# chennachaos/PFEMFort

Measured on AMD Instinct MI355X. Metric: DOF/s (assembly+CG-to-tol), higher is better.
Workload: dtype f64

## Files before the change

include/pfem_amd_diag.h:

```cpp
#ifndef PFEM_AMD_DIAG_H
#define PFEM_AMD_DIAG_H

#include "pfem_amd.h"

#ifdef __cplusplus
extern "C" {
#endif

#define PFEM_ASSEMBLY_GATHER 0
#define PFEM_ASSEMBLY_SCATTER 1
int pfem_solver_set_assembly_mode(pfem_solver *s, int mode);
int pfem_solver_assembly_info(pfem_solver *s, int *gather_form, int *hub_nodes, int *block_threads, int64_t *lds_bytes);
#define PFEM_SPMV_AUTO 0
#define PFEM_SPMV_INT32 1
#define PFEM_SPMV_GAPS16 2
#define PFEM_SPMV_GROUPED 3
int pfem_solver_set_spmv_format(pfem_solver *s, int format);
int pfem_solver_get_spmv_format(pfem_solver *s, int *bits_per_column);
int pfem_solver_get_spmv_row_group(pfem_solver *s, int *rows_per_lane);
int pfem_solver_get_spmv_gap_table(pfem_solver *s, int *entries);
int pfem_solver_get_spmv_value_dictionary(pfem_solver *s, int *entries);
int pfem_solver_amg_value_dictionaries(pfem_solver *s, int max_levels, int *n_levels, int *entries);
int pfem_solver_get_spmv_gap_escapes(pfem_solver *s, int *in_use);
int pfem_solver_spmv_bytes(pfem_solver *s, int64_t *format_bytes);

int pfem_solver_amg_info(pfem_solver *s, int max_levels, int *n_levels, int64_t *rows, int64_t *nnz, double *lambda_max,
                         double *symbolic_ms, double *numeric_ms, int *cheb_degree, int *fine_degree, double *eig_ratio, double *coarse_scale);
int pfem_solver_amg_aggregates(pfem_solver *s, int level, int32_t *agg);
int pfem_solver_amg_transfer(pfem_solver *s, int level, int *rbm, int *fine_bs, int *coarse_bs, int *dim, int64_t *n_nodes, double *node_xyz);
int pfem_solver_amg_layout(pfem_solver *s, int max_levels, int *coupled, int *distributed_levels, int64_t *first_dof, int64_t *local_rows);
int pfem_solver_incidence_patterns(pfem_solver *s, int *count, int *longest);
int pfem_solver_amg_aggregation(pfem_solver *s, int max_levels, int *n_levels, int *kind);
int pfem_solver_amg_comm_counts(pfem_solver *s, int *exchanges_per_cycle, int *allreduces_per_cycle);
int pfem_solver_amg_cycle_profile(pfem_solver *s, int max_levels, int *n_levels, int *exchanges, double *exchange_ms,
                                  int64_t *exchange_doubles, int *allreduces, double *allreduce_ms, int64_t *allreduce_doubles,
                                  double *cycle_ms);
int pfem_solver_amg_pairing(pfem_solver *s, int *lattice_levels);
int pfem_solver_amg_cycle(pfem_solver *s, int *cycle, int *last_level_visited_twice);
int pfem_solver_amg_level0_epilogue(pfem_solver *s, int *taken);

int pfem_eval_elems(pfem_solver *s, const double *elemData, const double *timeData,
                    double *K_out, double *F_out);

int pfem_matrix_info(pfem_solver *s, int64_t *n_owned, int64_t *n_local, int64_t *nnz,
                     int64_t *stored_entries);

int pfem_spmv(pfem_solver *s, const double *x, double *y);
int pfem_bench_spmv(pfem_solver *s, int reps, double *ms_per_launch);

typedef struct pfem_timings {
    double pattern_ms;
    double assemble_ms;
    double solve_ms;
    double spmv_ms_total;
    int64_t spmv_launches;
    double upload_ms;
    double event_overhead_ms;
    double iface_ms_total;
    double scalar_ms_total;
    int64_t comm_samples;
    double exposed_ms_total;
    int64_t graph_iterations;
// ... 21 lines not shown
```

pfemfort_amd/_lib.py:

```python
from __future__ import annotations

import ctypes as C
import os

_HERE = os.path.dirname(os.path.abspath(__file__))
LIB_PATH = os.environ.get("PFEM_AMD_LIB") or os.path.join(_HERE, "libpfem_amd.so")

OK, ERR_ARG, ERR_STATE, ERR_NEG_JAC, ERR_HIP, ERR_NOGPU, ERR_NOMEM, ERR_DIVERGED, ERR_PATTERN, ERR_COMM = range(10)
POISSON_TRIA, POISSON_TET, ELAST_TET, POISSON_TRIA_INLINE, ELAST_TRIA = 1, 2, 3, 4, 5
SOLVER_EMPTY, PATTERN_OK, INIT_OK, ASSEMBLY_OK, FACTORISE_OK = 1, 2, 3, 4, 5
INSERT_VALUES, ADD_VALUES = 1, 2

NPELEM = {POISSON_TRIA: 3, POISSON_TET: 4, ELAST_TET: 4, POISSON_TRIA_INLINE: 3, ELAST_TRIA: 3}
NDOF = {POISSON_TRIA: 1, POISSON_TET: 1, ELAST_TET: 3, POISSON_TRIA_INLINE: 1, ELAST_TRIA: 2}
NDIM = {POISSON_TRIA: 2, POISSON_TET: 3, ELAST_TET: 3, POISSON_TRIA_INLINE: 2, ELAST_TRIA: 2}


class PfemError(RuntimeError):
    def __init__(self, code: int, where: str, detail: str = ""):
        self.code = code
        msg = f"{where}: error {code} ({_strerror(code)})"
        if detail:
            msg += f" -- {detail}"
        super().__init__(msg)
# ... 68 lines not shown
    "pfem_solver_get_spmv_format": [_P, _P],
    "pfem_solver_get_spmv_row_group": [_P, _P],
    "pfem_solver_get_spmv_gap_table": [_P, _P],
    "pfem_solver_get_spmv_value_dictionary": [_P, _P],
    "pfem_solver_amg_value_dictionaries": [_P, _I, _P, _P],
    "pfem_solver_get_spmv_gap_escapes": [_P, _P],
    "pfem_solver_spmv_bytes": [_P, _P],
    "pfem_solver_set_preconditioner": [_P, _I],
    "pfem_solver_get_preconditioner": [_P, _P],
    "pfem_solver_set_cg_single_reduction": [_P, _I],
    "pfem_solver_amg_info": [_P, _I, _P, _P, _P, _P, _P, _P, _P, _P, _P, _P],
    "pfem_solver_amg_aggregates": [_P, _I, _P],
    "pfem_solver_amg_transfer": [_P, _I, _P, _P, _P, _P, _P, _P],
    "pfem_solver_amg_layout": [_P, _I, _P, _P, _P, _P],
    "pfem_solver_amg_aggregation": [_P, _I, _P, _P],
    "pfem_solver_incidence_patterns": [_P, _P, _P],
    "pfem_solver_amg_comm_counts": [_P, _P, _P],
    "pfem_solver_amg_cycle_profile": [_P, _I, _P, _P, _P, _P, _P, _P, _P, _P],
    "pfem_solver_amg_pairing": [_P, _P],
    "pfem_solver_set_amg_options": [_P, _I, _I, _D, _D],
    "pfem_solver_set_amg_cycle": [_P, _I],
    "pfem_solver_amg_cycle": [_P, _P, _P],
    "pfem_solver_amg_level0_epilogue": [_P, _P],
    "pfem_eval_elems": [_P, _P, _P, _P, _P],
    "pfem_rhs_add_values": [_P, _L, _P, _P],
    "pfem_matrix_info": [_P, _P, _P, _P, _P],
    "pfem_get_local_to_global": [_P, _P],
    "pfem_get_csr": [_P, _P, _P, _P],
    "pfem_get_rhs": [_P, _P],
    "pfem_spmv": [_P, _P, _P],
    "pfem_bench_spmv": [_P, _I, _P],
    "pfem_get_timings": [_P, _P],
    "pfem_solver_profile_spmv": [_P, _I],
    "pfem_neighbour_plan": [_I, _I, _P, _P, _P, _P, _P, _P, _P, _P, _P],
    "pfem_solver_set_neighbours": [_P, _I, _P, _P, _P],
    "pfem_rccl_unique_id": [_P],
    "pfem_solver_set_comm_rccl": [_P, _I, _I, _P],
    "pfem_solver_set_comm_host": [_P, _I, _I, HOST_ALLREDUCE_FN, HOST_EXCHANGE_FN, _P],
    "pfem_solver_comm_bench": [_P, C.c_int64, _I, _P, _P],
    "pfem_solver_comm_bench_sizes": [_P, C.c_int64, C.c_int64, _I, _I, _P, _P],
    "pfem_solver_set_comm_peer": [_P, _I, _I, HOST_ALLREDUCE_FN, HOST_EXCHANGE_FN, _P],
    "pfem_solver_comm_shutdown": [_P],
    "pfem_solver_comm_info": [_P, _P, _P, _P, _P],
    "pfem_solver_comm_describe": [_P, _P, _I, _P, _P, _P, _P, _P],
    "pfem_solver_comm_selftest": [_P, _L, _P],
    "pfem_get_ghosts": [_P, _P, _P],
# ... 53 lines not shown
```

pfemfort_amd/csrc/pfem_amg.inc:

```

constexpr int kAmgMaxLevels = 14;
constexpr int kAmgMatchRounds = 8;
constexpr int kAmgPasses = 3;
constexpr int64_t kAmgReplicateRows = 150000;
constexpr int kAmgRetryBlock = -7701;

inline bool amg_in_effect(const pfem_solver *s)
{
    return s->pc == PFEM_PC_GAMG;
}

inline SellDev amg_sell(const pfem_solver *s, const AmgLevel &L, int64_t rows)
{
    SellDev A;
    if (L.fine) {
        A = s->sell();
    } else {
        A.slice_off = L.slice_off.p;
        A.rowlen = L.rowlen.p;
        A.cols = L.cols.p;
        A.vals = L.vals.p;
    }
    A.n_rows = rows;
    A.n_slices = (rows + 63) / 64;
// ... 527 lines not shown
    const size_t n = static_cast<size_t>(std::max<int64_t>(L.n_loc, 1));
    const size_t g = L.fine ? static_cast<size_t>(kVecGuard) : 0;
    const size_t nv = n;
    PFEM_TRY(L.dinv.alloc(n));
    PFEM_TRY(L.t.alloc(nv));
    PFEM_TRY(L.r.alloc(n));
    if (!L.fine) PFEM_TRY(L.b.alloc(n));
    PFEM_TRY(L.x_store.alloc(nv + 2 * g));
    PFEM_TRY(L.dd_store.alloc(nv + 2 * g));
    PFEM_HIP(hipMemsetAsync(L.x_store.p, 0, sizeof(double) * (nv + 2 * g), s->stream));
    PFEM_HIP(hipMemsetAsync(L.dd_store.p, 0, sizeof(double) * (nv + 2 * g), s->stream));
    L.x = L.x_store.p + g;
    L.dd = L.dd_store.p + g;
    PFEM_TRY(L.lam.alloc(1));
    PFEM_TRY(L.part_max.alloc(static_cast<size_t>(grid_for((L.n_loc + 63) / 64 * 64))));
    return PFEM_OK;
}

inline bool amg_galerkin_by_entry()
{
    static const bool v = std::getenv("PFEM_AMG_GALERKIN_MAPS") != nullptr;
    return v;
}
inline void amg_galerkin(pfem_solver *s, const AmgLevel &L, AmgLevel &C, const SellDev &A, bool extras = false, VdState *vstate = nullptr)
{
    C.bound_fresh = C.vd_direct = false;
    if (L.code_of.p && !amg_galerkin_by_entry()) {
        if (C.n_loc < 1) return;
        LatGalExtra X{nullptr, nullptr, nullptr, nullptr, nullptr};
        if (extras && C.dinv.p && C.t.p && C.n_loc == C.n) {
            X.dinv_out = C.dinv.p;
            X.ratio_out = C.t.p;
            C.bound_fresh = true;
            if (vstate && C.vd_have_dict && C.vd_hash_ok && C.vhash.p && C.vcodes.p && C.vcodes.n >= static_cast<size_t>(C.stored) && !C.vd_refused) {
                const VdState reset{C.vd_n, 0, 0, 0};
                (void)hipMemcpyAsync(vstate, &reset, sizeof reset, hipMemcpyHostToDevice, s->stream);
                X.vhash = C.vhash.p;
                X.codes = C.vcodes.p;
                X.vstate = vstate;
                C.vd_direct = true;
            }
        }
        hipLaunchKernelGGL(k_lat_galerkin, dim3(static_cast<unsigned>((C.n_loc + kLatGalThreads - 1) / kLatGalThreads)), dim3(kLatGalThreads), 0, s->stream, A, C.n_loc,
                           static_cast<const int32_t *>(L.mem_ptr.p), static_cast<const int32_t *>(L.mem_idx.p), static_cast<const uint8_t *>(L.code_of.p),
                           static_cast<const uint32_t *>(L.code_mask.p), static_cast<const int64_t *>(C.slice_off.p), C.vals.p, X);
        return;
    }
    hipLaunchKernelGGL(k_amg_galerkin, dim3(grid_for(L.nnz_c)), dim3(kBlock), 0, s->stream, L.nnz_c, static_cast<const int64_t *>(L.src_ptr.p),
                       static_cast<const int32_t *>(L.src_slot.p), static_cast<const int64_t *>(L.dst_slot.p),
                       static_cast<const double *>(A.vals), C.vals.p);
}

int amg_couple_level(pfem_solver *s, AmgWork &W, AmgLevel &L, AmgLevel &C, bool overlap, int cb, const std::vector<double> *nc_of)
{
    std::vector<int64_t> rank_off;
    if (cb > 0 && nc_of) {
        rank_off.assign(nc_of->size() + 1, 0);
        for (size_t q = 0; q < nc_of->size(); ++q) rank_off[q + 1] = rank_off[q] + static_cast<int64_t>((*nc_of)[q]);
    }
    auto node_base = [&](int64_t g) -> int64_t {
        const size_t q = static_cast<size_t>(std::upper_bound(rank_off.begin(), rank_off.end(), g) - rank_off.begin()) - 1;
        return rank_off[q] + (g - rank_off[q]) / cb * cb;
    };
    const PlanRef P = amg_plan(s, L);
// ... 1985 lines not shown
        PFEM_TRY(check_kernel("k_vd_hash_build (coarse level)"));
        PFEM_TRY(encode(L, l));
    }
    PFEM_TRY(read_states());
    for (int l : build) {
        AmgLevel &L = *M.lev[static_cast<size_t>(l)];
        const VdState &v = st[static_cast<size_t>(l)];
        if (v.fail || v.count < 1 || v.count > kVdMax || v.miss) {
            L.vd_ok = L.vd_have_dict = L.vd_hash_ok = false;
            L.vd_refused = true;
        } else {
            L.vd_n = v.count;
            L.vd_have_dict = true;
            L.vd_ok = true;
            L.vd_hash_ok = L.vhash.p != nullptr;
        }
        if (std::getenv("PFEM_VD_VERBOSE"))
            std::fprintf(stderr, "  value dictionary, level %d: %d distinct values among %lld slots%s\n", l, v.count, static_cast<long long>(L.stored),
                         L.vd_ok ? "" : " -- the level keeps its fp64 values");
    }
    return PFEM_OK;
}

int amg_numeric(pfem_solver *s, Amg &M, bool overlap)
{
    if (M.coupled) return amg_numeric_coupled(s, M, overlap);
    const bool fresh = M.galerkin_fresh;
    M.galerkin_fresh = false;
    for (size_t l = 0; l < M.lev.size(); ++l) {
        AmgLevel &L = *M.lev[l];
        const SellDev A = amg_sell(s, L);
        if (l + 1 < M.lev.size() && !fresh) {
            AmgLevel &C = *M.lev[l + 1];
            if (L.rbm) amg_rbm_galerkin(s, L, C, A);
            else amg_galerkin(s, L, C, A, !M.rbm && !M.coupled, M.vd_states.p ? M.vd_states.p + (l + 1) : nullptr);
        }
        const unsigned g = grid_for(A.n_slices * 64);
        if (!L.fine && L.bound_fresh && !fresh) {
            L.bound_fresh = false;
            if (L.n > 65536) {
                const unsigned gm = std::min<unsigned>(g, 512u);
                hipLaunchKernelGGL(k_amg_max_rows, dim3(gm), dim3(kBlock), 0, s->stream, static_cast<const double *>(L.t.p), L.n, L.part_max.p);
                hipLaunchKernelGGL(k_amg_max, dim3(1), dim3(1024), 0, s->stream, static_cast<const double *>(L.part_max.p), static_cast<int64_t>(gm), L.lam.p);
            } else {
                hipLaunchKernelGGL(k_amg_max, dim3(1), dim3(1024), 0, s->stream, static_cast<const double *>(L.t.p), L.n, L.lam.p);
            }
            continue;
        }
        if (L.fine && s->asm_bound_fresh && &M == s->amg.get()) {
            const unsigned gm = std::min<unsigned>(g, 2048u);
            hipLaunchKernelGGL(k_amg_max_rows, dim3(gm), dim3(kBlock), 0, s->stream, static_cast<const double *>(L.t.p), L.n, L.part_max.p);
            hipLaunchKernelGGL(k_amg_max, dim3(1), dim3(1024), 0, s->stream, static_cast<const double *>(L.part_max.p), static_cast<int64_t>(gm), L.lam.p);
            s->asm_bound_fresh = false;
        } else {
        hipLaunchKernelGGL(k_amg_diag_bound, dim3(g), dim3(kBlock), 0, s->stream, A, static_cast<int32_t>(L.n), L.dinv.p, L.part_max.p);
        hipLaunchKernelGGL(k_amg_max, dim3(1), dim3(1024), 0, s->stream, static_cast<const double *>(L.part_max.p), static_cast<int64_t>(g), L.lam.p);
        }
        if (M.rbm) {
// ... 549 lines not shown
```

pfemfort_amd/csrc/pfem_amg_kernels.hpp:

```cpp
#pragma once

namespace pfem {

__device__ __forceinline__ int64_t amg_edge_key(int32_t i, int32_t j, int32_t hi_, int32_t hj_, double w, double di, double dj)
{
    if (!(w < 0.0) || !(di > 0.0) || !(dj > 0.0)) return -1;
    const double s = -w / sqrt(di * dj);
    int b = static_cast<int>(floor(8.0 * log2(s))) + 2048;
    b = b < 1 ? 1 : (b > 4095 ? 4095 : b);
    const int64_t lo = hi_ < hj_ ? hi_ : hj_, hi = hi_ < hj_ ? hj_ : hi_;
    const int64_t close = 0x7fffffffLL - (hi - lo);
    const int64_t par = (lo & 1) == 0;
    const int64_t a = i < j ? i : j, c = i < j ? j : i;
    const int64_t h = ((a * 2654435761LL + c * 40503LL) >> 7) & 0x7ffffLL;
    return (static_cast<int64_t>(b) << 51) | (close << 20) | (par << 19) | h;
}

__global__ void __launch_bounds__(kBlock) k_amg_match_pick(int64_t n, const int64_t *__restrict__ gptr, const int32_t *__restrict__ gcol,
                                                            const double *__restrict__ gw, const double *__restrict__ gdiag,
                                                            const int32_t *__restrict__ hint ,
                                                            const int32_t *__restrict__ match, int32_t *__restrict__ cand)
{
    const int64_t i = static_cast<int64_t>(blockIdx.x) * kBlock + threadIdx.x;
    if (i >= n) return;
// ... 406 lines not shown
    if (MAPS && I == na - 1) src_ptr[e] = p0 + run;
    uint32_t mask = 0;
    for (int32_t m = mem_ptr[I]; m < mem_ptr[I + 1]; ++m) {
        const int64_t i = mem_idx[m];
        const int64_t base = A.slice_off[i >> 6] + (i & 63);
        const int len = A.rowlen[i];
        for (int k = 0; k < len; ++k) {
            const int64_t q = base + 64LL * k;
            const int c = lat_code(B, pos[A.cols[q]], bix, biy, biz);
            if (MAPS) src_slot[p0 + at[c][t]++] = static_cast<int32_t>(q);
            code_of[q] = static_cast<uint8_t>(c);
            mask |= 1u << c;
        }
    }
    code_mask[I] = mask;
}
constexpr int kLatGalThreads = 128;
struct LatGalExtra {
    double *dinv_out, *ratio_out;
    const VdHashEntry *vhash;
    uint16_t *codes;
    VdState *vstate;
};
__global__ void __launch_bounds__(kLatGalThreads) k_lat_galerkin(SellDev A, int64_t na, const int32_t *__restrict__ mem_ptr,
                                                                  const int32_t *__restrict__ mem_idx, const uint8_t *__restrict__ code_of,
                                                                  const uint32_t *__restrict__ code_mask, const int64_t *__restrict__ c_slice_off,
                                                                  double *__restrict__ coarse_vals, LatGalExtra X)
{
    __shared__ double acc[kLatCodes][kLatGalThreads];
    const int64_t I = static_cast<int64_t>(blockIdx.x) * kLatGalThreads + threadIdx.x;
    if (I >= na) return;
    const int t = threadIdx.x;
#pragma unroll
    for (int c = 0; c < kLatCodes; ++c) acc[c][t] = 0.0;
    const int32_t m0 = mem_ptr[I], m1 = mem_ptr[I + 1];
    for (int32_t mb = m0; mb < m1; mb += 8) {
        int32_t mi[8];
        int len[8];
        int64_t base[8];
#pragma unroll
        for (int j = 0; j < 8; ++j) mi[j] = mb + j < m1 ? __builtin_nontemporal_load(mem_idx + mb + j) : -1;
#pragma unroll
        for (int j = 0; j < 8; ++j) {
            len[j] = mi[j] >= 0 ? A.rowlen[mi[j]] : 0;
            base[j] = mi[j] >= 0 ? A.slice_off[mi[j] >> 6] + (mi[j] & 63) : 0;
        }
#pragma unroll
        for (int j = 0; j < 8; ++j) {
            for (int k0 = 0; k0 < len[j]; k0 += 16) {
                double v[16];
                uint8_t c[16];
#pragma unroll
                for (int e = 0; e < 16; ++e) {
                    const bool in = k0 + e < len[j];
                    const int64_t q = base[j] + 64LL * (k0 + e);
                    v[e] = in ? __builtin_nontemporal_load(A.vals + q) : 0.0;
                    c[e] = in ? __builtin_nontemporal_load(code_of + q) : static_cast<uint8_t>(0);
                }
#pragma unroll
                for (int e = 0; e < 16; ++e)
                    if (k0 + e < len[j]) acc[c[e]][t] += v[e];
            }
        }
    }
    const int64_t out0 = c_slice_off[I >> 6] + (I & 63);
    double *out = coarse_vals + out0;
    const uint32_t mask = code_mask[I];
    int r = 0;
    double sabs = 0.0;
    bool missed = false;
#pragma unroll
    for (int c = 0; c < kLatCodes; ++c)
        if (mask & (1u << c)) {
            const double v = acc[c][t];
            out[64LL * r] = v;
            sabs += fabs(v);
            if (X.vhash) {
                int code = vd_hash_find(X.vhash, static_cast<unsigned long long>(__double_as_longlong(v)));
                if (code < 0) { missed = true; code = 0; }
                X.codes[out0 + 64LL * r] = static_cast<uint16_t>(code);
            }
            ++r;
        }
    if (X.dinv_out) {
        const double d = (mask & (1u << 13)) ? acc[13][t] : 0.0;
        const bool pos = d > 0.0;
        X.dinv_out[I] = pos ? 1.0 / d : 1.0;
        X.ratio_out[I] = pos ? sabs / d : 1.0;
    }
    if (missed) X.vstate->miss = 1;
}
constexpr int kLatticeTable = 4096;
__global__ void __launch_bounds__(kBlock) k_amg_distinct(const double *__restrict__ c, int64_t n, unsigned long long *__restrict__ table,
                                                          int *__restrict__ overflow)
{
    const int64_t i = static_cast<int64_t>(blockIdx.x) * kBlock + threadIdx.x;
    const double v = (i < n ? c[i] : 0.0) + 0.0;
    const unsigned long long key = static_cast<unsigned long long>(__double_as_longlong(v));
    const unsigned long long left = __shfl_up(key, 1, 64);
    if (i >= n || ((threadIdx.x & 63) != 0 && left == key && i - 1 < n)) return;
    if (key == ~0ull) { *overflow = 1; return; }
    unsigned h = static_cast<unsigned>((key * 0x9E3779B97F4A7C15ull) >> 52) & (kLatticeTable - 1);
    for (int probe = 0; probe < kLatticeTable; ++probe) {
        if ((probe & 63) == 0 && __hip_atomic_load(overflow, __ATOMIC_RELAXED, __HIP_MEMORY_SCOPE_AGENT) != 0) return;
        const unsigned long long cur = table[h];
        if (cur == key) return;
        if (cur == ~0ull) {
            const unsigned long long old = atomicCAS(&table[h], ~0ull, key);
            if (old == ~0ull || old == key) return;
        }
        h = (h + 1) & (kLatticeTable - 1);
    }
    *overflow = 1;
// ... 1341 lines not shown
```

pfemfort_amd/csrc/pfem_amg_types.hpp:

```cpp
#pragma once

struct AmgPlan {
    std::vector<int> peers;
    std::vector<int64_t> peer_off{0};
    std::vector<int32_t> send_lidx;
    int64_t n_send = 0, n_sh = 0;
    DevBuf<int32_t> d_send_lidx, d_sh_lidx, d_sh_ptr, d_sh_src;
    DevBuf<int32_t> d_row_sh;
};

struct AmgLevel {
    int64_t n = 0, n_slices = 0, stored = 0, nnz = 0;
    int64_t n_loc = 0;
    int64_t gid_off = 0;
    std::vector<int64_t> ghost_gid;
    AmgPlan plan;
    DevBuf<int32_t> gid;
    bool fine = false;
    DevBuf<int64_t> slice_off, rowptr;
    DevBuf<int32_t> rowlen, cols;
    DevBuf<double> vals;
    int bs = 1;
    int64_t n_nodes = 0;
    DevBuf<int32_t> node_of, comp_of;
// ... 4 lines not shown
    bool lat_global = false;
    std::vector<int> lat_cuts[3];
    std::vector<char> lat_single[3];
    int lat_shift[3] = {0, 0, 0};
    int lat_occ[6] = {0, 0, 0, 0, 0, 0};
    int lat_box[6] = {0, 0, 0, 0, 0, 0};
    bool lat_full = false;
    int lat_tlo[3] = {0, 0, 0}, lat_thi[3] = {0, 0, 0};
    bool lat_nodes_global = false;
    std::vector<std::pair<int, int>> lat_str[3];
    bool lat_split = false;
    std::vector<double> lat_coord;
    DevBuf<double> xyz;
    int agg_kind = 0;
    int64_t nc = 0;
    DevBuf<int32_t> agg;
    DevBuf<int32_t> mem_ptr, mem_idx;
    int64_t nnz_c = 0;
    DevBuf<int64_t> src_ptr;
    DevBuf<int32_t> src_slot;
    DevBuf<int64_t> dst_slot;
    DevBuf<uint8_t> code_of;
    DevBuf<uint32_t> code_mask;
    int dim = 0;
    bool rbm = false;
    DevBuf<double> cen;
    DevBuf<double> roff;
    DevBuf<int32_t> node_agg;
    DevBuf<int64_t> gptr;
    DevBuf<int32_t> gcol, brow;
    int64_t nblk = 0;
    DevBuf<double> dinv, t, r, b, x_store, dd_store, lam, part_max;
    DevBuf<uint16_t> vcodes;
    DevBuf<double> vdict;
    DevBuf<unsigned long long> vtable;
    int vd_n = 0;
    bool vd_ok = false, vd_have_dict = false, vd_refused = false;
    DevBuf<VdHashEntry> vhash;
    bool vd_hash_ok = false;
    bool vd_direct = false;
    bool bound_fresh = false;
    double *x = nullptr, *dd = nullptr;
    DevBuf<double> x1;
    double lam_host = 0.0;
};

// ... 4 lines not shown
    bool symbolic_ok = false;
    bool galerkin_fresh = false;
    double symbolic_ms = 0.0, numeric_ms = 0.0;
    int cheb_degree = 2;
    int fine_degree = 1;
    bool eig_ratio_given = false;
    bool coarse_scale_given = false;
    double eig_ratio_opt = 0.0, coarse_scale_opt = 0.0;
    double eig_ratio_auto = 16.0, coarse_scale_auto = 1.5;
    double eig_ratio = 8.0, coarse_scale = 1.5;
    CgGraph graph;
    hipEvent_t ev_num0 = nullptr, ev_num1 = nullptr;
    ~Amg()
    {
        if (ev_num0) (void)hipEventDestroy(ev_num0);
        if (ev_num1) (void)hipEventDestroy(ev_num1);
    }
    int tail_from = -1;
    size_t tail_lds_allowed = 0;
    int cycle_gamma = 1, w_to = -1;
    bool cycle_given = false;
    bool fused = true;
    bool level0_ep = false;
    int coarsest_sweeps = 8;
    bool coupled = false;
    bool coupled_fused = true;
    bool coupled_refused = false;
    int64_t n_last_global = 0;
    DevBuf<double> dense_glob, bx_glob, lam_all;
    std::unique_ptr<Amg> rep;
    DevBuf<double> rep_buf;
    DevBuf<int32_t> rep_pack_slot;
    int64_t rep_total = 0, rep_off = 0, rep_mine = 0;
    bool rbm = false;
    DevBuf<double> lam2;
    DevBuf<VdState> vd_states;
    int cycle_exchanges = 0, cycle_allreduces = 0;
};
```

pfemfort_amd/csrc/pfem_device.hip:

```cpp
#include <hip/hip_runtime.h>
#include <hip/hip_ext.h>
#include <hipcub/hipcub.hpp>
#include <rccl/rccl.h>
#include <dlfcn.h>

#include <algorithm>
#include <chrono>
#include <climits>
#include <cmath>
#include <cstdio>
#include <cstdlib>
#include <cstring>
#include <mutex>
#include <thread>
#include <string>
#include <deque>
#include <functional>
#include <map>
#include <memory>
#include <vector>

#include "pfem_internal.hpp"
#include "pfem_vdhash.hpp"
#include "pfem_kernels.hpp"
// ... 478 lines not shown
    bool use_grouped() const
    {
        return grouped && (spmv_format == PFEM_SPMV_GROUPED || (spmv_format == PFEM_SPMV_AUTO && n_groups >= min_groups_auto()));
    }
    bool relgrouped = false;
    bool rel_gap32 = false;
    bool rel_dict = false;
    DevBuf<uint32_t> d_gap_table;
    bool row_dict = false;
    DevBuf<uint32_t> d_row_gap_table;
    int64_t n_rgroups = 0, n_rslices = 0, r_stored = 0;
    DevBuf<int32_t> d_rcol0;
    DevBuf<int64_t> d_rslice_off, d_rslice_doff;
    DevBuf<uint32_t> d_rdwords;
    DevBuf<double> d_rvals;
    DevBuf<uint8_t> d_relk;
    bool rel_vals_current = false;
    bool asm_bound_fresh = false;
    DevBuf<int32_t> d_row_group;
    bool grp_vals_current = false;
    DevBuf<unsigned long long> d_vcodes, d_vtable;
    DevBuf<VdHashEntry> d_vhash;
    bool vd_hash_ok = false, vd_direct_pending = false;
    VdState vd_direct_verdict{0, 0, 1, 0};
    DevBuf<double> d_vdict;
    DevBuf<VdState> d_vstate;
    int vd_rows = 0, vd_n = 0;
    bool vd_current = false, vd_ok = false, vd_have_dict = false;
    double vd_encode_ms = 0.0;
    DevBuf<uint16_t> d_dcodes;
    DevBuf<double> d_ddict;
    DevBuf<unsigned long long> d_dtable;
    DevBuf<VdState> d_dstate;
    bool dinv_codes = false;
    DinvView dinv_view() const
    {
        return dinv_codes ? DinvView{d_dinv.p, d_dcodes.p, d_ddict.p, reinterpret_cast<const int *>(d_dstate.p)}
                          : DinvView{d_dinv.p, nullptr, nullptr, nullptr};
    }
    bool use_rel() const
    {
        return relgrouped && !use_grouped() &&
               (spmv_format == PFEM_SPMV_GROUPED || (spmv_format == PFEM_SPMV_AUTO && n_rgroups >= min_groups_auto()));
    }
    SellRDev sellr() const
    {
// ... 1808 lines not shown
    PFEM_HIP(hipcub::DeviceScan::ExclusiveSum(temp.p, tb3, words.p, s->d_gslice_doff.p, nsl, s->stream));
    int64_t tot_e = 0, tot_w = 0;
    PFEM_HIP(hipMemcpyAsync(&tot_e, s->d_gslice_off.p + s->n_gslices, sizeof(int64_t), hipMemcpyDeviceToHost, s->stream));
    PFEM_HIP(hipMemcpyAsync(&tot_w, s->d_gslice_doff.p + s->n_gslices, sizeof(int64_t), hipMemcpyDeviceToHost, s->stream));
    PFEM_HIP(hipStreamSynchronize(s->stream));
    s->g_stored = tot_e;
    PFEM_TRY(s->d_gcol0.alloc(static_cast<size_t>(s->n_gslices) * 64));
    s->g_gap_words = tot_w;
    PFEM_TRY(s->d_gdwords.alloc(static_cast<size_t>(std::max<int64_t>(tot_w, 1))));
    PFEM_TRY(s->d_gvals.alloc(static_cast<size_t>(std::max<int64_t>(tot_e, 1)) * kGroupRows));
    PFEM_HIP(hipMemsetAsync(s->d_err.p, 0, sizeof(int), s->stream));
    hipLaunchKernelGGL(k_group_cols_fill, dim3(grid_for(s->n_gslices * 64)), dim3(kBlock), 0, s->stream, s->sell(),
                       static_cast<const int32_t *>(s->d_group_row0.p), s->n_groups, s->n_gslices,
                       static_cast<const int64_t *>(s->d_gslice_off.p), static_cast<const int64_t *>(s->d_gslice_doff.p),
                       s->d_gcol0.p, s->d_gdwords.p, s->row_dict ? static_cast<const uint32_t *>(s->d_row_gap_table.p) : nullptr, s->d_err.p);
    PFEM_TRY(check_kernel("k_group_cols_fill"));
    int miss = 0;
    PFEM_TRY(fetch_err(s, &miss));
    PFEM_HIP(hipMemsetAsync(s->d_err.p, 0, sizeof(int), s->stream));
    PFEM_HIP(hipStreamSynchronize(s->stream));
    s->grouped = miss == 0;
    s->grp_vals_current = false;
    s->vd_current = s->vd_ok = s->vd_have_dict = s->vd_refused = false;
    s->vd_hash_ok = s->vd_direct_pending = false;
    s->vd_rows = 0;
    s->d_row_group.release();
    if (s->grouped) {
        PFEM_TRY(s->d_row_group.alloc(static_cast<size_t>(n)));
        hipLaunchKernelGGL(k_row_group_index, dim3(grid_for(s->n_groups)), dim3(kBlock), 0, s->stream, static_cast<const int32_t *>(s->d_group_row0.p),
                           s->n_groups, s->d_row_group.p);
        PFEM_TRY(check_kernel("k_row_group_index"));
        PFEM_HIP(hipMemsetAsync(s->d_gvals.p, 0, sizeof(double) * static_cast<size_t>(std::max<int64_t>(tot_e, 1)) * kGroupRows, s->stream));
        PFEM_HIP(hipStreamSynchronize(s->stream));
    }
    return PFEM_OK;
}

int build_rel_groups(pfem_solver *s)
{
    s->relgrouped = false;
    s->rel_gap32 = false;
    s->rel_dict = false;
    const int64_t n = s->n_loc;
    if (s->grouped || n < kRelRows || n > INT_MAX - kRelRows) return PFEM_OK;
    s->n_rgroups = (n + kRelRows - 1) / kRelRows;
    s->n_rslices = (s->n_rgroups + 63) / 64;
    DevBuf<int64_t> entries, words;
// ... 58 lines not shown
#define PFEM_REL_FILL(MODE)                                                                                                       \
    hipLaunchKernelGGL(k_rel_cols_fill<MODE>, dim3(grid_for(s->n_rslices * 64)), dim3(kBlock), 0, s->stream, s->sell(), s->n_rgroups, \
                       s->n_rslices, static_cast<const int64_t *>(s->d_rslice_off.p),                                             \
                       static_cast<const int64_t *>(s->d_rslice_doff.p), s->d_rcol0.p, s->d_rdwords.p,                            \
                       static_cast<const uint32_t *>(s->d_gap_table.p), s->d_err.p)
    PFEM_HIP(hipMemsetAsync(s->d_err.p, 0, sizeof(int), s->stream));
    if (gap32) PFEM_REL_FILL(kGap32);
    else if (dict) PFEM_REL_FILL(kGapDict16);
    else PFEM_REL_FILL(kGapLit16);
#undef PFEM_REL_FILL
    PFEM_TRY(check_kernel("k_rel_cols_fill"));
    int miss = 0;
    PFEM_TRY(fetch_err(s, &miss));
    PFEM_HIP(hipMemsetAsync(s->d_err.p, 0, sizeof(int), s->stream));
    PFEM_HIP(hipStreamSynchronize(s->stream));
    if (miss) return PFEM_OK;
    s->relgrouped = true;
    s->rel_gap32 = gap32;
    s->rel_dict = dict;
    s->rel_vals_current = false;
    s->asm_bound_fresh = false;
    s->vd_direct_pending = false;
    s->vd_current = s->vd_ok = s->vd_have_dict = s->vd_refused = false;
    s->vd_hash_ok = s->vd_direct_pending = false;
    s->vd_rows = 0;
    s->d_relk.release();
    if (s->max_row_len > 0) {
        PFEM_TRY(s->d_relk.alloc(static_cast<size_t>(std::max<int64_t>(s->stored, 1))));
        PFEM_HIP(hipMemsetAsync(s->d_relk.p, 0xff, static_cast<size_t>(std::max<int64_t>(s->stored, 1)), s->stream));
        PFEM_HIP(hipMemsetAsync(s->d_rvals.p, 0, sizeof(double) * static_cast<size_t>(std::max<int64_t>(tot_e, 1)) * kRelRows, s->stream));
        PFEM_HIP(hipMemsetAsync(s->d_err.p, 0, sizeof(int), s->stream));
        const dim3 vg(static_cast<unsigned>(s->n_rslices));
        if (gap32) hipLaunchKernelGGL(k_rel_slot_map<kGap32>, vg, dim3(kBlock), 0, s->stream, s->sell(), s->sellr(), s->d_relk.p, s->d_err.p);
        else if (dict) hipLaunchKernelGGL(k_rel_slot_map<kGapDict16>, vg, dim3(kBlock), 0, s->stream, s->sell(), s->sellr(), s->d_relk.p, s->d_err.p);
        else hipLaunchKernelGGL(k_rel_slot_map<kGapLit16>, vg, dim3(kBlock), 0, s->stream, s->sell(), s->sellr(), s->d_relk.p, s->d_err.p);
        PFEM_TRY(check_kernel("k_rel_slot_map"));
        int wide = 0;
        PFEM_TRY(fetch_err(s, &wide));
        PFEM_HIP(hipMemsetAsync(s->d_err.p, 0, sizeof(int), s->stream));
        if (wide) s->d_relk.release();
    }
    return PFEM_OK;
}

inline void mark_group_vals(pfem_solver *s)
{
    const bool vd_on = valdict_enabled();
// ... 62 lines not shown
        if (st.miss) {
            s->vd_ok = s->vd_have_dict = false;
            s->vd_refused = true;
            if (verbose) std::fprintf(stderr, "  value dictionary: a value of the collection pass is missing from its own dictionary, the SpMV keeps its fp64 copy\n");
            return PFEM_OK;
        }
    }
    s->vd_ok = true;
    s->vd_current = true;
    s->vd_hash_ok = rows == kRelRows && s->d_vhash.p != nullptr;
    s->vd_encode_ms = std::chrono::duration<double, std::milli>(std::chrono::steady_clock::now() - t0).count();
    if (verbose) std::fprintf(stderr, "  value dictionary: %d distinct values among %lld slots, codes refreshed in %.3f ms (host, incl. the wait)\n", s->vd_n,
                              static_cast<long long>(rows * n_entries), s->vd_encode_ms);
    return PFEM_OK;
}

int refresh_group_vals_only(pfem_solver *s);
int refresh_group_vals(pfem_solver *s)
{
    if (s->vd_direct_pending) {
        s->vd_direct_pending = false;
        const bool enabled = valdict_enabled();
        const VdState st = s->vd_direct_verdict;
        if (enabled && !st.miss && !st.fail && s->use_rel() && s->vd_rows == kRelRows) {
            s->vd_ok = s->vd_current = true;
            s->group_vals_stale = false;
            if (std::getenv("PFEM_VD_VERBOSE")) std::fprintf(stderr, "  value dictionary: codes written by the assembly kernel (%d values)\n", s->vd_n);
            return PFEM_OK;
        }
        s->vd_current = false;
        s->group_vals_stale = true;
    }
    PFEM_TRY(refresh_group_vals_only(s));
    return refresh_value_codes(s);
}
int refresh_group_vals_only(pfem_solver *s)
{
    if (s->use_rel() && s->group_vals_stale) {
        s->vd_current = false;
        const dim3 vg(static_cast<unsigned>(s->n_rslices));
        if (s->rel_gap32) hipLaunchKernelGGL(k_rel_vals<kGap32>, vg, dim3(kBlock), 0, s->stream, s->sell(), s->sellr(), s->d_rvals.p);
        else if (s->rel_dict) hipLaunchKernelGGL(k_rel_vals<kGapDict16>, vg, dim3(kBlock), 0, s->stream, s->sell(), s->sellr(), s->d_rvals.p);
        else hipLaunchKernelGGL(k_rel_vals<kGapLit16>, vg, dim3(kBlock), 0, s->stream, s->sell(), s->sellr(), s->d_rvals.p);
        PFEM_TRY(check_kernel("k_rel_vals"));
        s->group_vals_stale = false;
        return PFEM_OK;
    }
    if (!s->use_grouped() || !s->group_vals_stale) return PFEM_OK;
    s->vd_current = false;
    hipLaunchKernelGGL(k_group_vals, dim3(grid_for(s->n_gslices * 64)), dim3(kBlock), 0, s->stream, s->sell(), s->sellg(),
                       s->d_gvals.p);
    PFEM_TRY(check_kernel("k_group_vals"));
    s->group_vals_stale = false;
    return PFEM_OK;
// ... 2098 lines not shown
        entries[(*n_levels)++] = r.L->fine ? ((s->vd_ok && s->vd_current) ? s->vd_n : 0) : (r.L->vd_ok ? r.L->vd_n : 0);
    }
    return PFEM_OK;
}

extern "C" int pfem_solver_set_amg_cycle(pfem_solver *s, int cycle)
{
    if (!s || cycle < 0 || cycle > 2) return PFEM_ERR_ARG;
    if (!s->amg) s->amg.reset(new (std::nothrow) Amg());
    if (!s->amg) return PFEM_ERR_NOMEM;
    s->amg->cycle_given = cycle != 0;
    if (cycle != 0) s->amg->cycle_gamma = cycle;
    s->amg->graph.invalidate();
    return PFEM_OK;
}
extern "C" int pfem_solver_amg_level0_epilogue(pfem_solver *s, int *taken)
{
    if (!s || !taken) return PFEM_ERR_ARG;
    if (!s->amg || !s->amg->symbolic_ok) return PFEM_ERR_STATE;
    *taken = s->amg->level0_ep ? 1 : 0;
    return PFEM_OK;
}

extern "C" int pfem_solver_amg_cycle(pfem_solver *s, int *cycle, int *last_level_visited_twice)
{
    if (!s || !cycle || !last_level_visited_twice) return PFEM_ERR_ARG;
    if (!s->amg || !s->amg->symbolic_ok) return PFEM_ERR_STATE;
    const Amg &M = *s->amg;
    *cycle = M.cycle_gamma;
    *last_level_visited_twice = M.cycle_gamma > 1 ? std::min(M.w_to, static_cast<int>(M.lev.size()) - 2) : 0;
    return PFEM_OK;
}
```

pfemfort_amd/solver.py:

```python
from __future__ import annotations

import ctypes as C

import numpy as np

from . import _lib as L
from ._lib import (ADD_VALUES, ASSEMBLY_OK, FACTORISE_OK, INIT_OK, INSERT_VALUES,
                   PATTERN_OK, SOLVER_EMPTY)


def _p(a):
    return None if a is None else a.ctypes.data_as(C.c_void_p)


def _f64(a):
    return np.ascontiguousarray(a, dtype=np.float64)


def _i32(a):
    return np.ascontiguousarray(a, dtype=np.int32)


class PetscSolver:

# ... 205 lines not shown
            out["xyz"] = a
        return out

    def incidencePatterns(self):
        n = C.c_int(0); m = C.c_int(0)
        L.check(L.lib().pfem_solver_incidence_patterns(self._h, C.byref(n), C.byref(m)), "pfem_solver_incidence_patterns")
        return n.value, m.value

    def amgAggregation(self):
        mx = 32
        nl = C.c_int(0)
        kind = (C.c_int * mx)()
        L.check(L.lib().pfem_solver_amg_aggregation(self._h, mx, C.byref(nl), kind), "pfem_solver_amg_aggregation")
        names = {0: "none", 1: "bricks", 2: "node-bricks", 3: "split-bricks", 4: "lattice-passes", 5: "matching"}
        return [names.get(kind[l], str(kind[l])) for l in range(max(nl.value - 1, 0))]

    def amgInfo(self):
        mx = 32
        nl = C.c_int(0); rows = (C.c_int64 * mx)(); nnz = (C.c_int64 * mx)(); lam = (C.c_double * mx)()
        sym = C.c_double(0); num = C.c_double(0); deg = C.c_int(0); fdeg = C.c_int(0); ratio = C.c_double(0); scale = C.c_double(0)
        L.check(L.lib().pfem_solver_amg_info(self._h, mx, C.byref(nl), rows, nnz, lam, C.byref(sym), C.byref(num), C.byref(deg),
                                             C.byref(fdeg), C.byref(ratio), C.byref(scale)), "pfem_solver_amg_info")
        n = nl.value
        return {"levels": n, "rows": list(rows[:n]), "nnz": list(nnz[:n]), "lambda_max": list(lam[:n]), "symbolic_ms": sym.value,
                "numeric_ms": num.value, "cheb_degree": deg.value, "fine_degree": fdeg.value, "eig_ratio": ratio.value, "coarse_scale": scale.value}

    def amgAggregates(self, level, n_rows):
        a = np.empty(n_rows, np.int32)
        L.check(L.lib().pfem_solver_amg_aggregates(self._h, level, _p(a)), "pfem_solver_amg_aggregates")
        return a

    def amgLayout(self):
        mx = 32
        cp, nd = C.c_int(0), C.c_int(0)
        first = np.zeros(mx, np.int64)
        loc = np.zeros(mx, np.int64)
        L.check(L.lib().pfem_solver_amg_layout(self._h, mx, C.byref(cp), C.byref(nd), _p(first), _p(loc)), "pfem_solver_amg_layout")
        nl = self.amgInfo()["levels"]
        ex, ar = C.c_int(0), C.c_int(0)
        L.check(L.lib().pfem_solver_amg_comm_counts(self._h, C.byref(ex), C.byref(ar)), "pfem_solver_amg_comm_counts")
        lat = C.c_int(0)
        L.check(L.lib().pfem_solver_amg_pairing(self._h, C.byref(lat)), "pfem_solver_amg_pairing")
        return {"coupled": bool(cp.value), "distributed_levels": nd.value, "first_dof": first[:nl].tolist(), "local_rows": loc[:nl].tolist(),
                "exchanges_per_cycle": ex.value, "allreduces_per_cycle": ar.value, "lattice_levels": lat.value}

    def amgCycleProfile(self):
        mx = 32
        nl, na = C.c_int(0), C.c_int(0)
# ... 134 lines not shown
```

Before: 619.1 million.

## Sum level-1 Galerkin product from the SpMV's compressed value codes

Result: faster. 631.2 million, median of 6 (+2.0%).

```diff
diff --git a/include/pfem_amd_diag.h b/include/pfem_amd_diag.h
--- a/include/pfem_amd_diag.h
+++ b/include/pfem_amd_diag.h
@@ -38,6 +38,8 @@
 int pfem_solver_amg_pairing(pfem_solver *s, int *lattice_levels);
 int pfem_solver_amg_cycle(pfem_solver *s, int *cycle, int *last_level_visited_twice);
 int pfem_solver_amg_level0_epilogue(pfem_solver *s, int *taken);
+int pfem_solver_amg_galerkin_from_codes(pfem_solver *s, int *taken);
+int pfem_solver_amg_level_values(pfem_solver *s, int level, int64_t max_values, double *vals, int64_t *stored);
 
 int pfem_eval_elems(pfem_solver *s, const double *elemData, const double *timeData,
                     double *K_out, double *F_out);
diff --git a/pfemfort_amd/_lib.py b/pfemfort_amd/_lib.py
--- a/pfemfort_amd/_lib.py
+++ b/pfemfort_amd/_lib.py
@@ -114,6 +114,8 @@
     "pfem_solver_set_amg_cycle": [_P, _I],
     "pfem_solver_amg_cycle": [_P, _P, _P],
     "pfem_solver_amg_level0_epilogue": [_P, _P],
+    "pfem_solver_amg_galerkin_from_codes": [_P, _P],
+    "pfem_solver_amg_level_values": [_P, _I, _L, _P, _P],
     "pfem_eval_elems": [_P, _P, _P, _P, _P],
     "pfem_rhs_add_values": [_P, _L, _P, _P],
     "pfem_matrix_info": [_P, _P, _P, _P, _P],
diff --git a/pfemfort_amd/csrc/pfem_amg.inc b/pfemfort_amd/csrc/pfem_amg.inc
--- a/pfemfort_amd/csrc/pfem_amg.inc
+++ b/pfemfort_amd/csrc/pfem_amg.inc
@@ -573,7 +573,8 @@
     static const bool v = std::getenv("PFEM_AMG_GALERKIN_MAPS") != nullptr;
     return v;
 }
-inline void amg_galerkin(pfem_solver *s, const AmgLevel &L, AmgLevel &C, const SellDev &A, bool extras = false, VdState *vstate = nullptr)
+inline void amg_galerkin(pfem_solver *s, const AmgLevel &L, AmgLevel &C, const SellDev &A, bool extras = false, VdState *vstate = nullptr,
+                         bool from_codes = false)
 {
     C.bound_fresh = C.vd_direct = false;
     if (L.code_of.p && !amg_galerkin_by_entry()) {
@@ -591,6 +592,15 @@
                 X.vstate = vstate;
                 C.vd_direct = true;
             }
+        }
+        if (from_codes) {
+            hipLaunchKernelGGL(k_lat_galerkin_codes, dim3(static_cast<unsigned>((C.n_loc + kLatGalThreads - 1) / kLatGalThreads)), dim3(kLatGalThreads),
+                               sizeof(double) * static_cast<size_t>(std::max(s->vd_n, 1)), s->stream, C.n_loc, static_cast<const int32_t *>(L.mem_ptr.p),
+                               static_cast<const int32_t *>(L.mem_idx.p), static_cast<const int64_t *>(s->d_rslice_off.p),
+                               static_cast<const unsigned long long *>(s->d_vcodes.p), static_cast<const uint32_t *>(L.glat.p),
+                               static_cast<const double *>(s->d_vdict.p), s->vd_n, static_cast<const uint32_t *>(L.code_mask.p),
+                               static_cast<const int64_t *>(C.slice_off.p), C.vals.p, X);
+            return;
         }
         hipLaunchKernelGGL(k_lat_galerkin, dim3(static_cast<unsigned>((C.n_loc + kLatGalThreads - 1) / kLatGalThreads)), dim3(kLatGalThreads), 0, s->stream, A, C.n_loc,
                            static_cast<const int32_t *>(L.mem_ptr.p), static_cast<const int32_t *>(L.mem_idx.p), static_cast<const uint8_t *>(L.code_of.p),
@@ -2622,8 +2632,40 @@
     return PFEM_OK;
 }
 
+int amg_level0_codes(pfem_solver *s, Amg &M, AmgLevel &L, bool *yes)
+{
+    *yes = false;
+    const char *e = std::getenv("PFEM_AMG_GALERKIN_CODES");
+    if (e && std::atoi(e) == 0) return PFEM_OK;
+    if (&M != s->amg.get() || M.coupled || M.rbm || cg_multi(s) || !L.fine || L.rbm || L.bs != 1 || !L.code_of.p || !L.code_mask.p || amg_galerkin_by_entry() ||
+        s->n_hubs != 0 || L.stored != s->stored || L.glat_refused)
+        return PFEM_OK;
+    if (!valdict_enabled() || !s->use_rel() || s->rel_gap32 || s->vd_rows != kRelRows || !(s->vd_ok && s->vd_current && s->vd_have_dict) || s->vd_miss_step ||
+        s->vd_n < 1 || s->vd_n > kVdMax || !s->d_vcodes.p || !s->d_vdict.p || !s->d_relk.p || !s->d_rslice_off.p || s->r_stored < 1 ||
+        s->d_vcodes.n < static_cast<size_t>(s->r_stored))
+        return PFEM_OK;
+    if (!L.glat.p || L.glat_for != s->r_stored) {
+        PFEM_TRY(L.glat.alloc(static_cast<size_t>(s->r_stored)));
+        L.glat_for = -1;
+        PFEM_HIP(hipMemsetAsync(L.glat.p, 0xff, sizeof(uint32_t) * static_cast<size_t>(s->r_stored), s->stream));
+        PFEM_HIP(hipMemsetAsync(s->d_err.p, 0, sizeof(int), s->stream));
+        hipLaunchKernelGGL(k_lat_group_codes, dim3(grid_for(L.n)), dim3(kBlock), 0, s->stream, amg_sell(s, L), static_cast<const uint8_t *>(L.code_of.p),
+                           static_cast<const uint8_t *>(s->d_relk.p), static_cast<const int64_t *>(s->d_rslice_off.p), reinterpret_cast<uint8_t *>(L.glat.p),
+                           s->d_err.p);
+        PFEM_TRY(check_kernel("k_lat_group_codes"));
+        int bad = 0;
+        PFEM_TRY(fetch_err(s, &bad));
+        PFEM_HIP(hipMemsetAsync(s->d_err.p, 0, sizeof(int), s->stream));
+        if (bad) { L.glat.release(); L.glat_refused = true; return PFEM_OK; }
+        L.glat_for = s->r_stored;
+    }
+    *yes = true;
+    return PFEM_OK;
+}
+
 int amg_numeric(pfem_solver *s, Amg &M, bool overlap)
 {
+    M.galerkin_from_codes = false;
     if (M.coupled) return amg_numeric_coupled(s, M, overlap);
     const bool fresh = M.galerkin_fresh;
     M.galerkin_fresh = false;
@@ -2633,7 +2675,14 @@
         if (l + 1 < M.lev.size() && !fresh) {
             AmgLevel &C = *M.lev[l + 1];
             if (L.rbm) amg_rbm_galerkin(s, L, C, A);
-            else amg_galerkin(s, L, C, A, !M.rbm && !M.coupled, M.vd_states.p ? M.vd_states.p + (l + 1) : nullptr);
+            else {
+                bool from_codes = false;
+                if (l == 0) PFEM_TRY(amg_level0_codes(s, M, L, &from_codes));
+                amg_galerkin(s, L, C, A, !M.rbm && !M.coupled, M.vd_states.p ? M.vd_states.p + (l + 1) : nullptr, from_codes);
+                if (from_codes) M.galerkin_from_codes = true;
+                if (l == 0 && std::getenv("PFEM_VD_VERBOSE"))
+                    std::fprintf(stderr, "  gamg numeric: level 1 summed from %s\n", from_codes ? "the SpMV's value codes" : "the fp64 row form");
+            }
         }
         const unsigned g = grid_for(A.n_slices * 64);
         if (!L.fine && L.bound_fresh && !fresh) {
diff --git a/pfemfort_amd/csrc/pfem_amg_kernels.hpp b/pfemfort_amd/csrc/pfem_amg_kernels.hpp
--- a/pfemfort_amd/csrc/pfem_amg_kernels.hpp
+++ b/pfemfort_amd/csrc/pfem_amg_kernels.hpp
@@ -452,47 +452,9 @@
     uint16_t *codes;
     VdState *vstate;
 };
-__global__ void __launch_bounds__(kLatGalThreads) k_lat_galerkin(SellDev A, int64_t na, const int32_t *__restrict__ mem_ptr,
-                                                                  const int32_t *__restrict__ mem_idx, const uint8_t *__restrict__ code_of,
-                                                                  const uint32_t *__restrict__ code_mask, const int64_t *__restrict__ c_slice_off,
-                                                                  double *__restrict__ coarse_vals, LatGalExtra X)
-{
-    __shared__ double acc[kLatCodes][kLatGalThreads];
-    const int64_t I = static_cast<int64_t>(blockIdx.x) * kLatGalThreads + threadIdx.x;
-    if (I >= na) return;
-    const int t = threadIdx.x;
-#pragma unroll
-    for (int c = 0; c < kLatCodes; ++c) acc[c][t] = 0.0;
-    const int32_t m0 = mem_ptr[I], m1 = mem_ptr[I + 1];
-    for (int32_t mb = m0; mb < m1; mb += 8) {
-        int32_t mi[8];
-        int len[8];
-        int64_t base[8];
-#pragma unroll
-        for (int j = 0; j < 8; ++j) mi[j] = mb + j < m1 ? __builtin_nontemporal_load(mem_idx + mb + j) : -1;
-#pragma unroll
-        for (int j = 0; j < 8; ++j) {
-            len[j] = mi[j] >= 0 ? A.rowlen[mi[j]] : 0;
-            base[j] = mi[j] >= 0 ? A.slice_off[mi[j] >> 6] + (mi[j] & 63) : 0;
-        }
-#pragma unroll
-        for (int j = 0; j < 8; ++j) {
-            for (int k0 = 0; k0 < len[j]; k0 += 16) {
-                double v[16];
-                uint8_t c[16];
-#pragma unroll
-                for (int e = 0; e < 16; ++e) {
-                    const bool in = k0 + e < len[j];
-                    const int64_t q = base[j] + 64LL * (k0 + e);
-                    v[e] = in ? __builtin_nontemporal_load(A.vals + q) : 0.0;
-                    c[e] = in ? __builtin_nontemporal_load(code_of + q) : static_cast<uint8_t>(0);
-                }
-#pragma unroll
-                for (int e = 0; e < 16; ++e)
-                    if (k0 + e < len[j]) acc[c[e]][t] += v[e];
-            }
-        }
-    }
+__device__ __forceinline__ void lat_galerkin_row_out(const double (&acc)[kLatCodes][kLatGalThreads], int t, int64_t I, const uint32_t *__restrict__ code_mask,
+                                                     const int64_t *__restrict__ c_slice_off, double *__restrict__ coarse_vals, const LatGalExtra &X)
+{
     const int64_t out0 = c_slice_off[I >> 6] + (I & 63);
     double *out = coarse_vals + out0;
     const uint32_t mask = code_mask[I];
@@ -519,6 +481,125 @@
         X.ratio_out[I] = pos ? sabs / d : 1.0;
     }
     if (missed) X.vstate->miss = 1;
+}
+__global__ void __launch_bounds__(kLatGalThreads) k_lat_galerkin(SellDev A, int64_t na, const int32_t *__restrict__ mem_ptr,
+                                                                  const int32_t *__restrict__ mem_idx, const uint8_t *__restrict__ code_of,
+                                                                  const uint32_t *__restrict__ code_mask, const int64_t *__restrict__ c_slice_off,
+                                                                  double *__restrict__ coarse_vals, LatGalExtra X)
+{
+    __shared__ double acc[kLatCodes][kLatGalThreads];
+    const int64_t I = static_cast<int64_t>(blockIdx.x) * kLatGalThreads + threadIdx.x;
+    if (I >= na) return;
+    const int t = threadIdx.x;
+#pragma unroll
+    for (int c = 0; c < kLatCodes; ++c) acc[c][t] = 0.0;
+    const int32_t m0 = mem_ptr[I], m1 = mem_ptr[I + 1];
+    for (int32_t mb = m0; mb < m1; mb += 8) {
+        int32_t mi[8];
+        int len[8];
+        int64_t base[8];
+#pragma unroll
+        for (int j = 0; j < 8; ++j) mi[j] = mb + j < m1 ? __builtin_nontemporal_load(mem_idx + mb + j) : -1;
+#pragma unroll
+        for (int j = 0; j < 8; ++j) {
+            len[j] = mi[j] >= 0 ? A.rowlen[mi[j]] : 0;
+            base[j] = mi[j] >= 0 ? A.slice_off[mi[j] >> 6] + (mi[j] & 63) : 0;
+        }
+#pragma unroll
+        for (int j = 0; j < 8; ++j) {
+            for (int k0 = 0; k0 < len[j]; k0 += 16) {
+                double v[16];
+                uint8_t c[16];
+#pragma unroll
+                for (int e = 0; e < 16; ++e) {
+                    const bool in = k0 + e < len[j];
+                    const int64_t q = base[j] + 64LL * (k0 + e);
+                    v[e] = in ? __builtin_nontemporal_load(A.vals + q) : 0.0;
+                    c[e] = in ? __builtin_nontemporal_load(code_of + q) : static_cast<uint8_t>(0);
+                }
+#pragma unroll
+                for (int e = 0; e < 16; ++e)
+                    if (k0 + e < len[j]) acc[c[e]][t] += v[e];
+            }
+        }
+    }
+    lat_galerkin_row_out(acc, t, I, code_mask, c_slice_off, coarse_vals, X);
+}
+constexpr int kLatGalChunk = 16;
+__global__ void __launch_bounds__(kBlock) k_lat_group_codes(SellDev A, const uint8_t *__restrict__ code_of, const uint8_t *__restrict__ relk,
+                                                             const int64_t *__restrict__ rslice_off, uint8_t *__restrict__ glat, int *__restrict__ bad)
+{
+    const int64_t r = static_cast<int64_t>(blockIdx.x) * kBlock + threadIdx.x;
+    if (r >= A.n_rows) return;
+    const int64_t base = A.slice_off[r >> 6] + (r & 63);
+    const int len = A.rowlen[r];
+    const int64_t g = r >> 2;
+    const int64_t off = rslice_off[g >> 6];
+    const int width = static_cast<int>((rslice_off[(g >> 6) + 1] - off) >> 6);
+    uint8_t *gp = glat + 4 * (off + (g & 63)) + (r & 3);
+    for (int k = 0; k < len; ++k) {
+        const int64_t q = base + 64LL * k;
+        const int u = relk[q];
+        if (u >= width) { *bad = 1; continue; }
+        gp[4LL * 64 * u] = code_of[q];
+    }
+}
+__global__ void __launch_bounds__(kLatGalThreads) k_lat_galerkin_codes(int64_t na, const int32_t *__restrict__ mem_ptr, const int32_t *__restrict__ mem_idx,
+                                                                        const int64_t *__restrict__ rslice_off, const unsigned long long *__restrict__ vcodes,
+                                                                        const uint32_t *__restrict__ glat, const double *__restrict__ dict, int nd,
+                                                                        const uint32_t *__restrict__ code_mask, const int64_t *__restrict__ c_slice_off,
+                                                                        double *__restrict__ coarse_vals, LatGalExtra X)
+{
+    __shared__ double acc[kLatCodes][kLatGalThreads];
+    extern __shared__ double lat_vd[];
+    const int64_t I = static_cast<int64_t>(blockIdx.x) * kLatGalThreads + threadIdx.x;
+    const int t = threadIdx.x;
+    const bool live = I < na;
+    const int32_t m0 = live ? mem_ptr[I] : 0, m1 = live ? mem_ptr[I + 1] : 0;
+    for (int i = t; i < nd; i += kLatGalThreads) lat_vd[i] = dict[i];
+#pragma unroll
+    for (int c = 0; c < kLatCodes; ++c) acc[c][t] = 0.0;
+    __syncthreads();
+    if (!live) return;
+    unsigned long long w[kLatGalChunk];
+    uint32_t lc[kLatGalChunk];
+    int64_t held = -1;
+    for (int32_t mb = m0; mb < m1; mb += 8) {
+        int32_t mi[8];
+        int width[8];
+        int64_t wb[8];
+#pragma unroll
+        for (int j = 0; j < 8; ++j) mi[j] = mb + j < m1 ? __builtin_nontemporal_load(mem_idx + mb + j) : -1;
+#pragma unroll
+        for (int j = 0; j < 8; ++j) {
+            const int64_t gs = mi[j] >= 0 ? mi[j] >> 8 : 0;
+            const int64_t o0 = rslice_off[gs], o1 = rslice_off[gs + 1];
+            width[j] = mi[j] >= 0 ? static_cast<int>((o1 - o0) >> 6) : 0;
+            wb[j] = o0 + ((mi[j] >> 2) & 63);
+        }
+#pragma unroll
+        for (int j = 0; j < 8; ++j) {
+            const int sh16 = 16 * (mi[j] & 3), sh8 = 8 * (mi[j] & 3);
+            for (int k0 = 0; k0 < width[j]; k0 += kLatGalChunk) {
+                if (wb[j] != held || k0 > 0) {
+#pragma unroll
+                    for (int e = 0; e < kLatGalChunk; ++e) {
+                        const bool in = k0 + e < width[j];
+                        const int64_t q = wb[j] + 64LL * (k0 + e);
+                        w[e] = in ? __builtin_nontemporal_load(vcodes + q) : 0ull;
+                        lc[e] = in ? __builtin_nontemporal_load(glat + q) : ~0u;
+                    }
+                    held = k0 == 0 ? wb[j] : -1;
+                }
+#pragma unroll
+                for (int e = 0; e < kLatGalChunk; ++e) {
+                    const uint32_t c = (lc[e] >> sh8) & 0xffu;
+                    if (c < static_cast<uint32_t>(kLatCodes)) acc[c][t] += lat_vd[(w[e] >> sh16) & 0xffffu];
+                }
+            }
+        }
+    }
+    lat_galerkin_row_out(acc, t, I, code_mask, c_slice_off, coarse_vals, X);
 }
 constexpr int kLatticeTable = 4096;
 __global__ void __launch_bounds__(kBlock) k_amg_distinct(const double *__restrict__ c, int64_t n, unsigned long long *__restrict__ table,
diff --git a/pfemfort_amd/csrc/pfem_amg_types.hpp b/pfemfort_amd/csrc/pfem_amg_types.hpp
--- a/pfemfort_amd/csrc/pfem_amg_types.hpp
+++ b/pfemfort_amd/csrc/pfem_amg_types.hpp
@@ -50,6 +50,9 @@
     DevBuf<int64_t> dst_slot;
     DevBuf<uint8_t> code_of;
     DevBuf<uint32_t> code_mask;
+    DevBuf<uint32_t> glat;
+    int64_t glat_for = -1;
+    bool glat_refused = false;
     int dim = 0;
     bool rbm = false;
     DevBuf<double> cen;
@@ -100,6 +103,7 @@
     bool cycle_given = false;
     bool fused = true;
     bool level0_ep = false;
+    bool galerkin_from_codes = false;
     int coarsest_sweeps = 8;
     bool coupled = false;
     bool coupled_fused = true;
diff --git a/pfemfort_amd/csrc/pfem_device.hip b/pfemfort_amd/csrc/pfem_device.hip
--- a/pfemfort_amd/csrc/pfem_device.hip
+++ b/pfemfort_amd/csrc/pfem_device.hip
@@ -524,6 +524,7 @@
     DevBuf<unsigned long long> d_vcodes, d_vtable;
     DevBuf<VdHashEntry> d_vhash;
     bool vd_hash_ok = false, vd_direct_pending = false;
+    bool vd_miss_step = false;
     VdState vd_direct_verdict{0, 0, 1, 0};
     DevBuf<double> d_vdict;
     DevBuf<VdState> d_vstate;
@@ -2378,7 +2379,7 @@
     s->grouped = miss == 0;
     s->grp_vals_current = false;
     s->vd_current = s->vd_ok = s->vd_have_dict = s->vd_refused = false;
-    s->vd_hash_ok = s->vd_direct_pending = false;
+    s->vd_hash_ok = s->vd_direct_pending = s->vd_miss_step = false;
     s->vd_rows = 0;
     s->d_row_group.release();
     if (s->grouped) {
@@ -2483,7 +2484,7 @@
     s->asm_bound_fresh = false;
     s->vd_direct_pending = false;
     s->vd_current = s->vd_ok = s->vd_have_dict = s->vd_refused = false;
-    s->vd_hash_ok = s->vd_direct_pending = false;
+    s->vd_hash_ok = s->vd_direct_pending = s->vd_miss_step = false;
     s->vd_rows = 0;
     s->d_relk.release();
     if (s->max_row_len > 0) {
@@ -2592,6 +2593,7 @@
         s->vd_direct_pending = false;
         const bool enabled = valdict_enabled();
         const VdState st = s->vd_direct_verdict;
+        s->vd_miss_step = st.miss || st.fail;
         if (enabled && !st.miss && !st.fail && s->use_rel() && s->vd_rows == kRelRows) {
             s->vd_ok = s->vd_current = true;
             s->group_vals_stale = false;
@@ -2600,6 +2602,8 @@
         }
         s->vd_current = false;
         s->group_vals_stale = true;
+    } else if (!s->vd_current) {
+        s->vd_miss_step = false;
     }
     PFEM_TRY(refresh_group_vals_only(s));
     return refresh_value_codes(s);
@@ -4744,6 +4748,28 @@
     return PFEM_OK;
 }
 
+extern "C" int pfem_solver_amg_galerkin_from_codes(pfem_solver *s, int *taken)
+{
+    if (!s || !taken) return PFEM_ERR_ARG;
+    *taken = (s->amg && s->amg->symbolic_ok && s->amg->galerkin_from_codes) ? 1 : 0;
+    return PFEM_OK;
+}
+extern "C" int pfem_solver_amg_level_values(pfem_solver *s, int level, int64_t max_values, double *vals, int64_t *stored)
+{
+    if (!s || !stored || level < 1 || max_values < 0 || (max_values > 0 && !vals)) return PFEM_ERR_ARG;
+    if (!s->amg || !s->amg->symbolic_ok) return PFEM_ERR_STATE;
+    const std::vector<AmgLevelRef> lev = amg_levels_of(*s->amg);
+    if (static_cast<size_t>(level) >= lev.size()) return PFEM_ERR_STATE;
+    const AmgLevel &L = *lev[static_cast<size_t>(level)].L;
+    *stored = L.stored;
+    const int64_t n = std::min<int64_t>(max_values, L.stored);
+    if (n < 1 || !L.vals.p) return PFEM_OK;
+    PFEM_TRY(use_device(s));
+    PFEM_HIP(hipStreamSynchronize(s->stream));
+    PFEM_HIP(hipMemcpy(vals, L.vals.p, sizeof(double) * static_cast<size_t>(n), hipMemcpyDeviceToHost));
+    return PFEM_OK;
+}
+
 extern "C" int pfem_solver_amg_cycle(pfem_solver *s, int *cycle, int *last_level_visited_twice)
 {
     if (!s || !cycle || !last_level_visited_twice) return PFEM_ERR_ARG;
diff --git a/pfemfort_amd/solver.py b/pfemfort_amd/solver.py
--- a/pfemfort_amd/solver.py
+++ b/pfemfort_amd/solver.py
@@ -251,8 +251,18 @@
         L.check(L.lib().pfem_solver_amg_info(self._h, mx, C.byref(nl), rows, nnz, lam, C.byref(sym), C.byref(num), C.byref(deg),
                                              C.byref(fdeg), C.byref(ratio), C.byref(scale)), "pfem_solver_amg_info")
         n = nl.value
+        gc = C.c_int(0)
+        L.check(L.lib().pfem_solver_amg_galerkin_from_codes(self._h, C.byref(gc)), "pfem_solver_amg_galerkin_from_codes")
         return {"levels": n, "rows": list(rows[:n]), "nnz": list(nnz[:n]), "lambda_max": list(lam[:n]), "symbolic_ms": sym.value,
-                "numeric_ms": num.value, "cheb_degree": deg.value, "fine_degree": fdeg.value, "eig_ratio": ratio.value, "coarse_scale": scale.value}
+                "numeric_ms": num.value, "cheb_degree": deg.value, "fine_degree": fdeg.value, "eig_ratio": ratio.value, "coarse_scale": scale.value,
+                "galerkin_from_codes": bool(gc.value)}
+
+    def amgLevelValues(self, level):
+        n = C.c_int64(0)
+        L.check(L.lib().pfem_solver_amg_level_values(self._h, level, 0, None, C.byref(n)), "pfem_solver_amg_level_values")
+        a = np.empty(n.value, np.float64)
+        L.check(L.lib().pfem_solver_amg_level_values(self._h, level, n.value, _p(a), C.byref(n)), "pfem_solver_amg_level_values")
+        return a
 
     def amgAggregates(self, level, n_rows):
         a = np.empty(n_rows, np.int32)
```
